# MGI-tech-bioinformatics/SuperPlus

Hardware: AMD Instinct MI355X
Metric: k-mers/s (DF createDict stage: trim + canonical k-mer count + solid filter + spectrum + adjacency) (higher is better)
Workload: dtype u64

## Files before the change

superplus_amd/csrc/dfk.hip:

```cpp
#include "../../include/dfk.h"
#include "dfk_kernels.h"

#include <algorithm>
#include <chrono>
#include <cstdarg>
#include <cstdio>
#include <cstdlib>
#include <cstring>
#include <atomic>
#include <fcntl.h>
#include <functional>
#include <new>
#include <string>
#include <sys/mman.h>
#include <sys/stat.h>
#include <unistd.h>
#include <condition_variable>
#include <memory>
#include <mutex>
#include <thread>
#include <vector>

using namespace dfk;

// ... 279 lines not shown
    DevBuf ctr; int rc = c->alloc(ctr, 32, "trim counters"); if (rc) return rc;
    HIP_TRY(hipMemsetAsync(ctr.p, 0, 32, c->stream));
    rc = c->alloc(c->good_len, sizeof(uint32_t) * in.n_reads, "goodLens", true); if (rc) return rc;
    if (in.n_reads) {
        unsigned grid = (unsigned)std::min<uint64_t>((in.n_reads + 255) / 256, 8192);
        hipLaunchKernelGGL(HIP_KERNEL_NAME(k_trim<K>), dim3(grid), dim3(256), 0, c->stream,
                           in.pq, in.pq_off, in.pq_bytes, in.base_off, in.packed_bytes, in.read_len, in.n_reads, c->cfg.min_qual, (uint32_t*)c->good_len.p,
                           (unsigned long long*)ctr.p, (unsigned int*)((char*)ctr.p + 8),
                           (unsigned long long*)((char*)ctr.p + 16));
        HIP_TRY(hipGetLastError());
    }
    uint64_t h[3] = {0, 0, 0};
    HIP_TRY(hipMemcpyAsync(h, ctr.p, 24, hipMemcpyDeviceToHost, c->stream));
    HIP_TRY(hipStreamSynchronize(c->stream));
    c->release(ctr);
    if ((uint32_t)h[1]) return fail(DFK_E_INPUT, "malformed input: an offset table is not monotone or runs past its array, a PQVec stream is broken, or its length differs from read_len");
    if (h[2] == 0) return fail(DFK_E_NOGOOD, "Looks like your input data have almost no good bases.");
    *n_inst = h[0];
    return 0;
}

int device_scan(dfk_ctx* c, const uint64_t* in, uint64_t* out, uint64_t n)
{
    constexpr uint64_t PER = (uint64_t)SCAN_THREADS * SCAN_ITEMS;
    if (n == 0) return 0;
    const uint64_t nblk = (n + PER - 1) / PER;
    if (nblk == 1) {
        hipLaunchKernelGGL(k_scan_blocks, dim3(1), dim3(SCAN_THREADS), 0, c->stream, in, out, n, (uint64_t*)nullptr);
        HIP_TRY(hipGetLastError());
        return 0;
    }
    DevBuf sums; int rc = c->alloc(sums, nblk * 8, "scan block sums"); if (rc) return rc;
    hipLaunchKernelGGL(k_scan_blocks, dim3((unsigned)nblk), dim3(SCAN_THREADS), 0, c->stream, in, out, n, (uint64_t*)sums.p);
    HIP_TRY(hipGetLastError());
    rc = device_scan(c, (const uint64_t*)sums.p, (uint64_t*)sums.p, nblk); if (rc) return rc;
    hipLaunchKernelGGL(k_scan_add, dim3((unsigned)nblk), dim3(SCAN_THREADS), 0, c->stream, out, n, (const uint64_t*)sums.p);
    HIP_TRY(hipGetLastError());
    HIP_TRY(hipStreamSynchronize(c->stream));
    c->release(sums);
    return 0;
}

struct BucketTable {
    uint32_t log2_nb = 0;
    DevBuf acc;
    DevBuf summ;
    DevBuf classes;
    DevBuf ovf_list; uint64_t n_ovf = 0;
    DevBuf class_hist;
    std::vector<uint64_t> h_class;
    uint64_t n_records = 0, n_inst = 0;
};
struct Partition {
    DevBuf records, base, ipre, items;
    uint64_t n_records = 0, n_inst = 0, n_items = 0;
    uint64_t nb = 0;
};

template <int K>
PartParams part_params(const dfk_ctx* c, uint32_t log2_nb, uint32_t log2_world, int64_t read_id0, uint32_t sub_lo, uint32_t sub_n)
{
    const uint32_t M = c->cfg.minimizer_len;
    return PartParams{M, (uint32_t)K - M + 1, log2_nb, log2_world, read_id0, sub_lo, sub_n,
                      sweep_class_mask(sub_lo, sub_n, log2_nb - log2_world)};
}

int table_totals(dfk_ctx* c, const DevBuf& acc, uint64_t nb, uint64_t* n_records, uint64_t* n_inst)
{
    DevBuf tot; int rc = c->alloc(tot, 16, "bucket totals"); if (rc) return rc;
    HIP_TRY(hipMemsetAsync(tot.p, 0, 16, c->stream));
    hipLaunchKernelGGL(k_sum_acc, dim3(1024), dim3(256), 0, c->stream, (const unsigned long long*)acc.p, nb, (unsigned long long*)tot.p);
    HIP_TRY(hipGetLastError());
    uint64_t h[2];
    HIP_TRY(hipMemcpyAsync(h, tot.p, 16, hipMemcpyDeviceToHost, c->stream));
    HIP_TRY(hipStreamSynchronize(c->stream));
    c->release(tot);
    *n_records = h[0]; *n_inst = h[1];
    return 0;
}

struct ScanJob {
    PartParams pp; uint64_t nb = 0, n_bins = 0, ovf_cap = 0; bool by_class = false, ranged = false;
    DevBuf ovf_tmp, d_n;
    std::vector<std::pair<hipEvent_t, hipEvent_t>> ev;
    ~ScanJob() { for (auto& e : ev) { (void)hipEventDestroy(e.first); (void)hipEventDestroy(e.second); } }
};

template <int K> bool scan_takes_ranges(const dfk_ctx* c) { return c->cfg.minimizer_len == 16; }

template <int K>
int scan_begin(dfk_ctx* c, const Inputs& in, uint32_t log2_world, int64_t read_id0, BucketTable* T, bool by_class, ScanJob* J)
{
    J->pp = part_params<K>(c, T->log2_nb, log2_world, read_id0, 0, 1u << (T->log2_nb - log2_world));
    J->nb = 1ull << T->log2_nb; J->by_class = by_class;
    int rc = 0;
    J->n_bins = 2ull * (PART_CLASSES << log2_world);
    if (by_class) { rc = c->alloc(T->class_hist, J->n_bins * 8, "class counters", true); if (rc) return rc; HIP_TRY(hipMemsetAsync(T->class_hist.p, 0, J->n_bins * 8, c->stream)); }
    else { rc = c->alloc(T->acc, J->nb * 8, "bucket counters", true); if (rc) return rc; }
    rc = c->alloc(T->summ, std::max<uint64_t>(1, in.n_reads) * 16, "run summaries", true); if (rc) return rc;
    rc = c->alloc(T->classes, std::max<uint64_t>(1, in.n_reads) * 4, "read bucket classes", true); if (rc) return rc;
    if (!by_class) HIP_TRY(hipMemsetAsync(T->acc.p, 0, J->nb * 8, c->stream));
    J->ovf_cap = in.n_reads / 16 + 1024;
    rc = c->alloc(J->ovf_tmp, J->ovf_cap * 4, "overflow read list (scratch)"); if (rc) return rc;
    rc = c->alloc(J->d_n, 16, "overflow read count"); if (rc) return rc;
    HIP_TRY(hipMemsetAsync(J->d_n.p, 0, 16, c->stream));
    return 0;
}

template <int K>
int scan_range(dfk_ctx* c, const Inputs& in, BucketTable* T, ScanJob* J, uint64_t r0, uint64_t r1)
{
    if (r1 <= r0) return 0;
    const PartParams& pp = J->pp;
    const bool by_class = J->by_class;
    unsigned grid = (unsigned)((r1 - r0 + PART_THREADS - 1) / PART_THREADS);
    static const unsigned scan_blocks = getenv("DFK_SCAN_BLOCKS") ? (unsigned)atoi(getenv("DFK_SCAN_BLOCKS")) : 0;
    if (by_class) grid = std::min<unsigned>(grid, (scan_blocks ? scan_blocks : 128u) * (unsigned)c->prop.multiProcessorCount);
    else if (scan_blocks) grid = std::min<unsigned>(grid, scan_blocks * (unsigned)c->prop.multiProcessorCount);
    const size_t lds_a = (sizeof(uint32_t) + 1) * pp.W * PART_THREADS + sizeof(uint32_t) * PART_RING * PART_THREADS + (by_class ? J->n_bins * 4 : 0);
    hipEvent_t e0, e1;
    HIP_TRY(hipEventCreate(&e0)); HIP_TRY(hipEventCreate(&e1));
    J->ev.emplace_back(e0, e1);
    HIP_TRY(hipEventRecord(e0, c->stream));
    if (scan_takes_ranges<K>(c)) {
        const size_t lds_r = sizeof(uint32_t) * (PART_RING + SUMMARY_RUNS) * PART_THREADS + (by_class ? J->n_bins * 4 : 0);
        hipLaunchKernelGGL(HIP_KERNEL_NAME(k_scan_count<K, 16>), dim3(grid), dim3(PART_THREADS), lds_r, c->stream,
                           in.packed, in.packed_bytes, in.base_off, (const uint32_t*)c->good_len.p, r0, r1, pp,
                           (unsigned long long*)T->acc.p, (unsigned long long*)T->class_hist.p, (unsigned long long*)J->d_n.p, J->ovf_cap,
                           (uint32_t*)J->ovf_tmp.p, (uint4*)T->summ.p, (uint32_t*)T->classes.p);
    } else {
        if (r0 != 0 || r1 != in.n_reads) return fail(DFK_E_STATE, "the general scan takes every read at once");
        hipLaunchKernelGGL(HIP_KERNEL_NAME(k_partition<K, false>), dim3(grid), dim3(PART_THREADS), lds_a, c->stream,
                           in.packed, in.packed_bytes, in.base_off, (const uint32_t*)c->good_len.p, in.bc,
                           (int64_t)c->cfg.ign_bc_below, in.n_reads, pp, (unsigned long long*)T->acc.p, (unsigned long long*)T->class_hist.p,
                           (unsigned long long*)J->d_n.p, J->ovf_cap, (uint4*)J->ovf_tmp.p, (uint4*)T->summ.p,
                           (const uint32_t*)nullptr, (uint64_t)0, (const uint64_t*)nullptr, (uint32_t*)T->classes.p);
    }
    HIP_TRY(hipGetLastError());
    HIP_TRY(hipEventRecord(e1, c->stream));
    return 0;
}

template <int K>
int scan_end(dfk_ctx* c, const Inputs& in, uint64_t n_inst, BucketTable* T, ScanJob* J)
{
    int rc = 0;
    T->n_ovf = 0;
    if (in.n_reads) {
        HIP_TRY(hipMemcpyAsync(&T->n_ovf, J->d_n.p, 8, hipMemcpyDeviceToHost, c->stream));
        HIP_TRY(hipStreamSynchronize(c->stream));
        if (T->n_ovf > J->ovf_cap) {
            c->release(J->ovf_tmp);
            rc = c->alloc(J->ovf_tmp, in.n_reads * 4, "overflow read list (scratch)"); if (rc) return rc;
            HIP_TRY(hipMemsetAsync(J->d_n.p, 0, 16, c->stream));
            hipLaunchKernelGGL(k_select_overflow, dim3((unsigned)std::min<uint64_t>((in.n_reads + 255) / 256, 8192)), dim3(256), 0, c->stream,
                               (const uint4*)T->summ.p, in.n_reads, (uint32_t*)J->ovf_tmp.p, (unsigned long long*)J->d_n.p);
            HIP_TRY(hipGetLastError());
            HIP_TRY(hipMemcpyAsync(&T->n_ovf, J->d_n.p, 8, hipMemcpyDeviceToHost, c->stream));
            HIP_TRY(hipStreamSynchronize(c->stream));
        }
        if (T->n_ovf) {
            rc = c->alloc(T->ovf_list, T->n_ovf * 4, "overflow read list", true); if (rc) return rc;
            HIP_TRY(hipMemcpyAsync(T->ovf_list.p, J->ovf_tmp.p, T->n_ovf * 4, hipMemcpyDeviceToDevice, c->stream));
            HIP_TRY(hipStreamSynchronize(c->stream));
        }
    }
    c->release(J->ovf_tmp); c->release(J->d_n);
    HIP_TRY(hipStreamSynchronize(c->stream));
    float ms = 0;
    for (auto& e : J->ev) { float m = 0; if (hipEventElapsedTime(&m, e.first, e.second) == hipSuccess) ms += m; }
    c->st.ms_part_count = ms; c->st.reserved[6] = J->ev.size();
    TRACE("%llu of %llu reads have more than %d runs", (unsigned long long)T->n_ovf, (unsigned long long)in.n_reads, SUMMARY_RUNS);
    if (J->by_class) {
        T->h_class.assign(J->n_bins, 0);
        HIP_TRY(hipMemcpyAsync(T->h_class.data(), T->class_hist.p, J->n_bins * 8, hipMemcpyDeviceToHost, c->stream));
        HIP_TRY(hipStreamSynchronize(c->stream));
        T->n_records = T->n_inst = 0;
        for (uint64_t i = 0; i < J->n_bins / 2; ++i) { T->n_records += T->h_class[i]; T->n_inst += T->h_class[J->n_bins / 2 + i]; }
    } else { rc = table_totals(c, T->acc, J->nb, &T->n_records, &T->n_inst); if (rc) return rc; }
    TRACE("partition count pass done (%llu buckets, %llu records%s)", (unsigned long long)J->nb, (unsigned long long)T->n_records, J->ev.size() > 1 ? ", in ranges under the upload" : "");
    if (T->n_inst != n_inst)
        return fail(DFK_E_HIP, "partition count pass saw %llu instances, trim saw %llu%s",
                    (unsigned long long)T->n_inst, (unsigned long long)n_inst,
                    (n_inst - T->n_inst) % (1ull << 32) == 0 ? " (a fine bucket with 2^32 or more instances: its counter keeps 32 bits)" : "");
    c->st.n_records = T->n_records; c->st.n_buckets = J->nb;
    return 0;
}

template <int K>
int partition_count(dfk_ctx* c, const Inputs& in, uint64_t n_inst, uint32_t log2_world, int64_t read_id0, BucketTable* T, bool by_class = false)
{
    ScanJob J;
    int rc = scan_begin<K>(c, in, log2_world, read_id0, T, by_class, &J); if (rc) return rc;
    rc = scan_range<K>(c, in, T, &J, 0, in.n_reads); if (rc) return rc;
    return scan_end<K>(c, in, n_inst, T, &J);
}

int pass_tables(dfk_ctx* c, const DevBuf& acc, uint32_t log2_sub, uint32_t world, uint32_t sub_lo, uint32_t sub_n, uint64_t budget, Partition* P)
{
    P->nb = (uint64_t)world * sub_n;
    const uint64_t nb = P->nb;
    DevBuf rec, inst, flags, idx;
    int rc = c->alloc(rec, (nb + 1) * 8, "bucket record counts"); if (rc) return rc;
    rc = c->alloc(inst, (nb + 1) * 8, "bucket instance counts"); if (rc) return rc;
    rc = c->alloc(P->base, (nb + 1) * 8, "bucket bases"); if (rc) return rc;
    rc = c->alloc(P->ipre, (nb + 1) * 8, "bucket instance prefix"); if (rc) return rc;
    const unsigned g1 = (unsigned)((nb + 1 + 255) / 256);
    hipLaunchKernelGGL(k_slice, dim3(g1), dim3(256), 0, c->stream, (const unsigned long long*)acc.p, log2_sub, sub_lo, sub_n, nb,
                       (uint64_t*)rec.p, (uint64_t*)inst.p);
    HIP_TRY(hipGetLastError());
    rc = device_scan(c, (const uint64_t*)rec.p, (uint64_t*)P->base.p, nb + 1); if (rc) return rc;
    rc = device_scan(c, (const uint64_t*)inst.p, (uint64_t*)P->ipre.p, nb + 1); if (rc) return rc;
    rc = c->alloc(flags, (nb + 1) * 8, "item flags"); if (rc) return rc;
    rc = c->alloc(idx, (nb + 1) * 8, "item index"); if (rc) return rc;
    hipLaunchKernelGGL(k_item_flags, dim3(g1), dim3(256), 0, c->stream, (const uint64_t*)P->ipre.p, nb, budget, (uint64_t*)flags.p);
    HIP_TRY(hipGetLastError());
    rc = device_scan(c, (const uint64_t*)flags.p, (uint64_t*)idx.p, nb + 1); if (rc) return rc;
    uint64_t tot[3];
    HIP_TRY(hipMemcpyAsync(&tot[0], (const uint64_t*)P->base.p + nb, 8, hipMemcpyDeviceToHost, c->stream));
    HIP_TRY(hipMemcpyAsync(&tot[1], (const uint64_t*)P->ipre.p + nb, 8, hipMemcpyDeviceToHost, c->stream));
    HIP_TRY(hipMemcpyAsync(&tot[2], (const uint64_t*)idx.p + nb, 8, hipMemcpyDeviceToHost, c->stream));
    HIP_TRY(hipStreamSynchronize(c->stream));
    P->n_records = tot[0]; P->n_inst = tot[1]; P->n_items = tot[2];
    rc = c->alloc(P->items, std::max<uint64_t>(1, P->n_items) * sizeof(ItemRange), "work items"); if (rc) return rc;
    hipLaunchKernelGGL(k_item_pairs, dim3((unsigned)((nb + 255) / 256)), dim3(256), 0, c->stream, (const uint64_t*)flags.p,
                       (const uint64_t*)idx.p, nb, (ItemRange*)P->items.p);
    HIP_TRY(hipGetLastError());
    HIP_TRY(hipStreamSynchronize(c->stream));
    c->release(rec); c->release(inst); c->release(flags); c->release(idx);
    return 0;
// ... 1641 lines not shown
```

superplus_amd/csrc/dfk_kernels.h:

```cpp
#pragma once
#include <type_traits>
#include "dfk_device.h"

namespace dfk {

template <int K>
__global__ void __launch_bounds__(256)
k_trim(const uint8_t* __restrict__ pq, const uint64_t* __restrict__ pq_off, uint64_t pq_nbytes,
       const uint64_t* __restrict__ base_off, uint64_t packed_bytes, const uint32_t* __restrict__ read_len,
       uint64_t n_reads, uint32_t min_qual, uint32_t* __restrict__ good_len,
       unsigned long long* __restrict__ n_inst, unsigned int* __restrict__ bad,
       unsigned long long* __restrict__ sum_good)
{
    unsigned long long mine = 0, good = 0;
    bool any_bad = false;
    for (uint64_t r = (uint64_t)blockIdx.x * blockDim.x + threadIdx.x; r < n_reads; r += (uint64_t)gridDim.x * blockDim.x) {
        uint32_t gl = 0;
        uint64_t p = pq_off[r], end = pq_off[r + 1];
        uint32_t idx = 0, run = 0;
        const uint64_t b0 = base_off[r], b1 = base_off[r + 1];
        bool ok = p <= end && end <= pq_nbytes && b0 <= b1 && b1 <= packed_bytes && b1 - b0 >= ((uint64_t)read_len[r] + 3) / 4;
        if (!ok) end = p;
        while (p < end) {
            uint32_t nQs = pq[p];
// ... 259 lines not shown
        }
        arr[bi * PART_THREADS + tid] = h;
        if (++bi == W) {
            uint32_t run = h, ri = W - 1;
            if (!WRITE) sidx[(W - 1) * PART_THREADS + tid] = (uint8_t)(W - 1);
            for (int i0 = (int)W - 2; i0 >= 0; i0 -= 8) {
                uint32_t v[8];
#pragma unroll
                for (int k = 0; k < 8; ++k) v[k] = i0 - k >= 0 ? arr[(i0 - k) * PART_THREADS + tid] : 0u;
#pragma unroll
                for (int k = 0; k < 8; ++k) {
                    const int i = i0 - k;
                    if (i >= 0) {
                        const bool lt = v[k] < run;
                        run = lt ? v[k] : run;
                        arr[i * PART_THREADS + tid] = run;
                        if (!WRITE) { ri = lt ? (uint32_t)i : ri; sidx[i * PART_THREADS + tid] = (uint8_t)ri; }
                    }
                }
            }
            bi = 0;
        }
        if (bi + 1 < W) sfx_next = arr[(bi + 1) * PART_THREADS + tid];
    }
    close_run();
    if (!WRITE) {
        const uint64_t lo = sum_lo | (qn <= (uint32_t)SUMMARY_RUNS ? qn : SUMMARY_OVERFLOW), hi = sum_hi;
        summaries[r] = uint4{(uint32_t)lo, (uint32_t)(lo >> 32), (uint32_t)hi, (uint32_t)(hi >> 32)};
        if (read_classes) read_classes[r] = cmask;
        if (qn > (uint32_t)SUMMARY_RUNS && bucket_cur) {
            const unsigned long long at = atomicAdd(bucket_cur, 1ull);
            if (at < n_out) reinterpret_cast<uint32_t*>(records)[at] = (uint32_t)r;
        }
    }
    if (WRITE) {
        for (uint32_t e = 0; e < qn; ++e) {
            uint32_t a = queue[(2 * e) * PART_THREADS + tid], b = queue[(2 * e + 1) * PART_THREADS + tid];
            const uint64_t dst = place(b);
            if (dst != ~0ull) emit_record<K>(words, n_words, bit0, a & 0xFFFFu, a >> 16, b, gl, tag, dst, records);
        }
    }
}

template <int K, bool WRITE>
__global__ void __launch_bounds__(PART_THREADS)
k_partition(const uint8_t* __restrict__ packed, uint64_t packed_bytes, const uint64_t* __restrict__ base_off,
            const uint32_t* __restrict__ good_len, const int32_t* __restrict__ bc, int64_t ign_bc_below,
            uint64_t n_reads, PartParams pp,
            unsigned long long* __restrict__ bucket_acc,
            unsigned long long* __restrict__ class_hist,
            unsigned long long* __restrict__ bucket_cur,
            uint64_t n_out,
            uint4* __restrict__ records,
            uint4* __restrict__ summaries,
            const uint32_t* __restrict__ read_list,
            uint64_t n_list,
            const uint64_t* __restrict__ slice_base,
            uint32_t* __restrict__ read_classes)
{
    extern __shared__ uint32_t smem[];
    uint32_t* lh = nullptr;
    const uint32_t n_bins = 2u * (PART_CLASSES << pp.log2_world);
    if (!WRITE && class_hist) {
        lh = reinterpret_cast<uint32_t*>(reinterpret_cast<uint8_t*>(smem) + 5 * pp.W * PART_THREADS + 4 * PART_RING * PART_THREADS);
        for (uint32_t i = threadIdx.x; i < n_bins; i += PART_THREADS) lh[i] = 0;
        __syncthreads();
    }
    const uint64_t n_work = (WRITE && read_list) ? n_list : n_reads;
    for (uint64_t r0 = (uint64_t)blockIdx.x * PART_THREADS; r0 < n_work; r0 += (uint64_t)gridDim.x * PART_THREADS)
        partition_read<K, WRITE>(r0 + threadIdx.x, smem, lh, packed, packed_bytes, base_off, good_len, bc, ign_bc_below, n_reads, pp,
                                 bucket_acc, bucket_cur, n_out, records, summaries, read_list, n_list, slice_base, read_classes);
    if (lh) {
        __syncthreads();
        for (uint32_t i = threadIdx.x; i < n_bins; i += PART_THREADS) if (lh[i]) atomicAdd(&class_hist[i], (unsigned long long)lh[i]);
    }
}

template <int I, int N, class F>
__device__ __forceinline__ void static_for(F&& f)
{
    if constexpr (I < N) { f(std::integral_constant<int, I>{}); static_for<I + 1, N>(f); }
}

template <int K, int M>
__global__ void __launch_bounds__(PART_THREADS)
k_scan_count(const uint8_t* __restrict__ packed, uint64_t packed_bytes, const uint64_t* __restrict__ base_off,
             const uint32_t* __restrict__ good_len, uint64_t r_first, uint64_t n_reads , PartParams pp,
             unsigned long long* __restrict__ bucket_acc, unsigned long long* __restrict__ class_hist,
             unsigned long long* __restrict__ ovf_count, uint64_t ovf_cap, uint32_t* __restrict__ ovf_list,
             uint4* __restrict__ summaries, uint32_t* __restrict__ read_classes)
{
    constexpr int W = K - M + 1;
    constexpr uint32_t mmask = M == 16 ? 0xFFFFFFFFu : ((1u << (2 * M)) - 1u);
    constexpr uint32_t rsh = 2 * (M - 1);
    constexpr int RUNS = SUMMARY_RUNS;
    extern __shared__ uint32_t smem[];
    uint32_t* ring = smem;
    uint32_t* runb = smem + PART_RING * PART_THREADS;
    uint32_t* lh = nullptr;
    const uint32_t n_bins = 2u * (PART_CLASSES << pp.log2_world);
    if (class_hist) {
        lh = runb + RUNS * PART_THREADS;
        for (uint32_t i = threadIdx.x; i < n_bins; i += PART_THREADS) lh[i] = 0;
        __syncthreads();
    }
    const int tid = threadIdx.x;
    const uint32_t* words = reinterpret_cast<const uint32_t*>(packed);
    const uint64_t n_words = (packed_bytes + 3) >> 2;
    const uint32_t log2_local = pp.log2_nb - pp.log2_world;
    for (uint64_t r0 = r_first + (uint64_t)blockIdx.x * PART_THREADS; r0 < n_reads; r0 += (uint64_t)gridDim.x * PART_THREADS) {
        const uint64_t r = r0 + tid;
        const uint32_t gl = r < n_reads ? good_len[r] : 0;
        const bool live = gl >= (uint32_t)K + 1;
        uint32_t qn = 0, cmask = 0;
        uint64_t sum_lo = 0, sum_hi = 0;
        if (live) {
            const uint64_t bit0 = base_off[r] * 8;
            uint64_t wi = bit0 >> 5, filled_to = wi;
            auto fill = [&]() {
                uint32_t w[PART_RING];
#pragma unroll
                for (int k = 0; k < PART_RING; ++k) w[k] = filled_to + k < n_words ? words[filled_to + k] : 0u;
#pragma unroll
                for (int k = 0; k < PART_RING; ++k) ring[((filled_to + k) & (PART_RING - 1)) * PART_THREADS + tid] = w[k];
                filled_to += PART_RING;
            };
            fill();
            uint32_t wbits = ring[(wi & (PART_RING - 1)) * PART_THREADS + tid], wpos = (uint32_t)bit0 & 31u;
            auto next_base = [&]() -> uint32_t {
                const uint32_t b = (wbits >> wpos) & 3u;
                wpos += 2;
                if (wpos == 32) { wpos = 0; ++wi; if (wi == filled_to) fill(); wbits = ring[(wi & (PART_RING - 1)) * PART_THREADS + tid]; }
                return b;
            };
            uint32_t f = 0, rc = 0;
            for (int j = 0; j < M - 1; ++j) { const uint32_t b = next_base(); f = ((f << 2) | b) & mmask; rc = (rc >> 2) | ((3u - b) << rsh); }
            const uint32_t n_mmers = gl - M + 1;
            uint32_t arr[W], sidxw[(W + 3) / 4];
            auto sidx_get = [&](int i) -> uint32_t { return (sidxw[i >> 2] >> (8 * (i & 3))) & 255u; };
            auto sidx_set = [&](int i, uint32_t v) { const uint32_t sh = 8u * (uint32_t)(i & 3); sidxw[i >> 2] = (sidxw[i >> 2] & ~(255u << sh)) | (v << sh); };
#pragma unroll
            for (int i = 0; i < (W + 3) / 4; ++i) sidxw[i] = 0;
            uint32_t P = 0, Pi = 0;
            uint32_t cur_b = 0, cur_nk = 0, cur_rel = 0;
            auto close_run = [&]() {
                if (qn < (uint32_t)RUNS) {
                    runb[qn * PART_THREADS + tid] = cur_b;
                    const uint64_t fld = cur_nk | (cur_rel << 6);
                    const uint32_t b = 8u + 12u * qn;
                    if (b < 64u) { sum_lo |= fld << b; if (b > 52u) sum_hi |= fld >> (64u - b); } else sum_hi |= fld << (b - 64u);
                } else {
                    if (lh) { const uint32_t bin = class_bin(cur_b, pp); atomicAdd(&lh[bin], 1u); atomicAdd(&lh[(PART_CLASSES << pp.log2_world) + bin], cur_nk); }
                    else atomicAdd(&bucket_acc[cur_b], (1ull << 32) | cur_nk);
                    cmask |= 1u << sweep_class_of(cur_b & ((1u << log2_local) - 1u), log2_local);
                }
                ++qn;
            };
            for (uint32_t t0 = 0; t0 < n_mmers; t0 += W) {
                static_for<0, W>([&](auto bi_c) {
                    constexpr int bi = decltype(bi_c)::value;
                    if (t0 + (uint32_t)bi < n_mmers) {
                        const uint32_t b = next_base();
                        f = ((f << 2) | b) & mmask;
                        rc = (rc >> 2) | ((3u - b) << rsh);
                        const uint32_t h = mmer_hash(f < rc ? f : rc);
                        const bool newmin = bi == 0 || h < P;
                        P = newmin ? h : P;
                        Pi = newmin ? (uint32_t)bi : Pi;
                        const bool first = t0 == 0;
                        if (!first || bi == W - 1) {
                            uint32_t mv = P;
                            bool older = false;
                            if constexpr (bi != W - 1) { older = arr[bi + 1] < mv; mv = older ? arr[bi + 1] : mv; }
                            const uint32_t bucket = bucket_of(mv, pp);
                            const bool open = first || bucket != cur_b || cur_nk == (uint32_t)KTraits<K>::NK_MAX;
                            if (open) {
                                if (!first) close_run();
                                cur_b = bucket; cur_nk = 1;
                                cur_rel = (bi != W - 1 && older) ? sidx_get(bi + 1 < W ? bi + 1 : 0) - (uint32_t)bi - 1u : (uint32_t)(W - 1 - bi) + Pi;
                            } else ++cur_nk;
                        }
                        arr[bi] = h;
                        if (bi == W - 1) {
                            uint32_t run = h, ri = W - 1;
                            sidx_set(W - 1, W - 1);
                            static_for<0, W - 1>([&](auto j_c) {
                                constexpr int i = W - 2 - decltype(j_c)::value;
                                const bool lt = arr[i] < run; run = lt ? arr[i] : run; arr[i] = run; ri = lt ? (uint32_t)i : ri; sidx_set(i, ri);
                            });
                        }
                    }
                });
            }
            close_run();
        }
        const uint32_t mine = min(qn, (uint32_t)RUNS);
        for (uint32_t i = 0; __ballot(i < mine) != 0ull; ++i) {
            if (i < mine) {
                const uint32_t cb = runb[i * PART_THREADS + tid];
                const uint32_t bfld = 8u + 12u * i;
                const uint32_t nk = (uint32_t)(bfld + 12 <= 64 ? sum_lo >> bfld : bfld >= 64 ? sum_hi >> (bfld - 64) : (sum_lo >> bfld) | (sum_hi << (64 - bfld))) & 63u;
                if (lh) { const uint32_t bin = class_bin(cb, pp); atomicAdd(&lh[bin], 1u); atomicAdd(&lh[(PART_CLASSES << pp.log2_world) + bin], nk); }
                else atomicAdd(&bucket_acc[cb], (1ull << 32) | nk);
                cmask |= 1u << sweep_class_of(cb & ((1u << log2_local) - 1u), log2_local);
            }
        }
        if (r < n_reads) {
            const uint64_t lo = sum_lo | (qn <= (uint32_t)SUMMARY_RUNS ? qn : SUMMARY_OVERFLOW);
            summaries[r] = uint4{(uint32_t)lo, (uint32_t)(lo >> 32), (uint32_t)sum_hi, (uint32_t)(sum_hi >> 32)};
            if (read_classes) read_classes[r] = cmask;
        }
        if (qn > (uint32_t)SUMMARY_RUNS) {
            const unsigned long long at = atomicAdd(ovf_count, 1ull);
            if (at < ovf_cap) ovf_list[at] = (uint32_t)r;
        }
    }
    if (lh) {
        __syncthreads();
        for (uint32_t i = threadIdx.x; i < n_bins; i += PART_THREADS) if (lh[i]) atomicAdd(&class_hist[i], (unsigned long long)lh[i]);
    }
}

constexpr int SLICE_READS = 16;
template <int K, bool EMIT, typename F>
__device__ __forceinline__ void for_each_run_in_pass(uint64_t r, const uint8_t* __restrict__ packed, uint64_t packed_bytes,
                                                     const uint64_t* __restrict__ base_off, const PartParams& pp,
                                                     const uint4* __restrict__ summaries, F&& f)
{
    const uint4 sm = summaries[r];
    const uint32_t n = sm.x & 15u;
    if (n == 0 || n == SUMMARY_OVERFLOW) return;
    const uint32_t* words = reinterpret_cast<const uint32_t*>(packed);
    const uint64_t n_words = (packed_bytes + 3) >> 2;
    const uint64_t bit0 = base_off[r] * 8;
    const uint32_t M = pp.M;
    const uint32_t mmask = M == 16 ? 0xFFFFFFFFu : ((1u << (2 * M)) - 1u);
    const uint64_t lo = (uint64_t)sm.x | ((uint64_t)sm.y << 32), hi = (uint64_t)sm.z | ((uint64_t)sm.w << 32);
    uint32_t s0 = 0;
#pragma unroll
    for (int i = 0; i < SUMMARY_RUNS; ++i) {
        if ((uint32_t)i < n) {
            constexpr int B0 = 8;
            const int b = B0 + 12 * i;
            const uint32_t fld = (uint32_t)(b + 12 <= 64 ? lo >> b : b >= 64 ? hi >> (b - 64) : (lo >> b) | (hi << (64 - b))) & 0xFFFu;
            const uint32_t nk = fld & 63u, rel = fld >> 6;
            const uint64_t bo = bit0 + 2ull * (s0 + rel);
            const uint64_t wi = bo >> 5;
            const uint32_t w0 = words[wi], w1 = wi + 1 < n_words ? words[wi + 1] : 0u;
            const uint32_t x = alignbit(w1, w0, (uint32_t)bo & 31u) & mmask;
            uint32_t y = __brev(x);
            y = ((y >> 1) & 0x55555555u) | ((y & 0x55555555u) << 1);
            const uint32_t fw = y >> (32 - 2 * M), rcv = ~x & mmask;
            const uint32_t bucket = bucket_of(mmer_hash(fw < rcv ? fw : rcv), pp);
            const uint32_t lb = pass_local(bucket, pp);
            if (lb != 0xFFFFFFFFu) f(s0, nk, lb, bucket >> (pp.log2_nb - pp.log2_world), bit0, (uint32_t)i + 1 == n);
            s0 += nk;
        }
    }
}

template <int K>
__global__ void __launch_bounds__(256)
k_scatter_slices(const uint8_t* __restrict__ packed, uint64_t packed_bytes, const uint64_t* __restrict__ base_off,
                 const uint32_t* __restrict__ good_len, const int32_t* __restrict__ bc, int64_t ign_bc_below,
                 uint64_t n_reads, PartParams pp, const uint4* __restrict__ summaries, const uint32_t* __restrict__ read_classes,
                 const uint64_t* __restrict__ slice_base,
                 unsigned long long* __restrict__ slice_fill,
                 uint4* __restrict__ records)
{
    __shared__ uint32_t cnt[256];
    __shared__ unsigned long long at[256];
    __shared__ uint16_t list[256 * SLICE_READS];
    __shared__ uint32_t n_list;
    const uint32_t world = 1u << pp.log2_world;
    const int lane = threadIdx.x & 63;
    const uint64_t r_block = (uint64_t)blockIdx.x * 256 * SLICE_READS;
    if (threadIdx.x < world) cnt[threadIdx.x] = 0;
    if (threadIdx.x == 0) n_list = 0;
    __syncthreads();
#pragma unroll
    for (int j = 0; j < SLICE_READS; ++j) {
        const uint32_t rel = 256u * j + threadIdx.x;
        const uint64_t r = r_block + rel;
        const bool hit = r < n_reads && (!read_classes || (read_classes[r] & pp.class_mask) != 0u);
        const unsigned long long mk = __ballot(hit);
        uint32_t w = 0;
        if (lane == 0 && mk) w = atomicAdd(&n_list, (uint32_t)__popcll(mk));
        w = __builtin_amdgcn_readfirstlane(w);
        if (hit) list[w + __popcll(mk & ((1ull << lane) - 1ull))] = (uint16_t)rel;
    }
    __syncthreads();
    const uint32_t n = n_list;
    for (uint32_t i = threadIdx.x; i < n; i += 256)
        for_each_run_in_pass<K, false>(r_block + list[i], packed, packed_bytes, base_off, pp, summaries,
                                       [&](uint32_t, uint32_t, uint32_t, uint32_t owner, uint64_t, bool) { atomicAdd(&cnt[owner], 1u); });
    __syncthreads();
    if (threadIdx.x < world) {
        const uint32_t m = cnt[threadIdx.x];
        at[threadIdx.x] = slice_base[threadIdx.x] + (m ? atomicAdd(&slice_fill[threadIdx.x], (unsigned long long)m) : 0ull);
        cnt[threadIdx.x] = 0;
    }
    __syncthreads();
    const uint32_t* words = reinterpret_cast<const uint32_t*>(packed);
// ... 1542 lines not shown
```

Baseline: 58.49 billion.

## Stage scan run keys by class and count via LDS sub-slice histograms

Instead of issuing a global 64-bit atomic per run into the bucket counter table, the ranged scan kernel stages run keys in LDS and flushes them into per-class global key arrays. A pipeline of follow-up kernels (sub-slice histogram, prefix scan, partition, per-sub-slice LDS count) then accumulates the bucket counters with shared-memory atomics and a single plain add per bucket. The aim is to remove scattered global atomic traffic over a large table. In exchange it adds multi-GB scratch buffers, extra block-wide synchronisation in the scan kernel, and several extra passes over the keys. It is only enabled when the estimated runs per read is at least 3.5.

```diff
diff --git a/superplus_amd/csrc/dfk.hip b/superplus_amd/csrc/dfk.hip
--- a/superplus_amd/csrc/dfk.hip
+++ b/superplus_amd/csrc/dfk.hip
@@ -385,6 +385,9 @@
 struct ScanJob {
     PartParams pp; uint64_t nb = 0, n_bins = 0, ovf_cap = 0; bool by_class = false, ranged = false;
     DevBuf ovf_tmp, d_n;
+    bool keyed = false; uint32_t n_cls = 0, n_sub = 0, sb = 0; uint64_t piece_reads = 0;
+    ScanKeys sk{};
+    DevBuf keys, keys2, fill, sub;
     std::vector<std::pair<hipEvent_t, hipEvent_t>> ev;
     ~ScanJob() { for (auto& e : ev) { (void)hipEventDestroy(e.first); (void)hipEventDestroy(e.second); } }
 };
@@ -407,6 +410,62 @@
     rc = c->alloc(J->ovf_tmp, J->ovf_cap * 4, "overflow read list (scratch)"); if (rc) return rc;
     rc = c->alloc(J->d_n, 16, "overflow read count"); if (rc) return rc;
     HIP_TRY(hipMemsetAsync(J->d_n.p, 0, 16, c->stream));
+    const double runs = in.n_reads ? 1.0 + 2.0 * std::max(0.0, 4.0 * (double)in.packed_bytes / (double)in.n_reads - K + 1) / (J->pp.W + 1) : 0.0;
+    J->keyed = !by_class && scan_takes_ranges<K>(c) && in.n_reads && (runs >= 3.5 || getenv("DFK_SCAN_KEY_PIECE"));
+    if (J->keyed) {
+        const uint32_t lb = T->log2_nb, cb = std::min<uint32_t>(6, lb);
+        J->sk.ib = lb - cb; J->n_cls = 1u << cb;
+        J->sb = std::min(KEY_SUB_BITS, J->sk.ib); J->n_sub = 1u << (J->sk.ib - J->sb);
+        const double per_read = 1.25 * runs;
+        constexpr uint64_t KEY_SCRATCH_MAX = 16ull << 30;
+        const uint64_t want = 8ull * (uint64_t)(per_read * (double)in.n_reads) + 8ull * J->n_cls;
+        const uint64_t room = std::min<uint64_t>(std::min(want, KEY_SCRATCH_MAX), c->largest_allocatable() / 3);
+        J->sk.cap = std::max<uint64_t>(1024, room / 8 / J->n_cls);
+        J->piece_reads = std::max<uint64_t>(PART_THREADS, (uint64_t)((double)(J->sk.cap * J->n_cls) / per_read));
+        if (const char* e = getenv("DFK_SCAN_KEY_PIECE")) J->piece_reads = std::max<uint64_t>(1, std::min<uint64_t>(J->piece_reads, strtoull(e, nullptr, 10)));
+        const uint64_t n_subs = (uint64_t)J->n_cls * J->n_sub;
+        rc = c->alloc(J->keys, J->sk.cap * J->n_cls * 4, "run keys (scratch)"); if (rc) return rc;
+        rc = c->alloc(J->keys2, J->sk.cap * J->n_cls * 4, "run keys by sub-slice (scratch)"); if (rc) return rc;
+        rc = c->alloc(J->fill, J->n_cls * 8, "run key slice fills (scratch)"); if (rc) return rc;
+        rc = c->alloc(J->sub, (3 * n_subs + 1) * 8, "run key sub-slices (scratch)"); if (rc) return rc;
+        J->sk.keys = (uint32_t*)J->keys.p; J->sk.fill = (unsigned long long*)J->fill.p;
+        TRACE("run keys: %u classes of %llu keys, %u sub-slices each, pieces of %llu reads", J->n_cls, (unsigned long long)J->sk.cap,
+              J->n_sub, (unsigned long long)J->piece_reads);
+    }
+    return 0;
+}
+
+template <int K>
+int scan_keys_piece(dfk_ctx* c, const Inputs& in, BucketTable* T, ScanJob* J, uint64_t r0, uint64_t r1)
+{
+    static const unsigned scan_blocks = getenv("DFK_SCAN_BLOCKS") ? (unsigned)atoi(getenv("DFK_SCAN_BLOCKS")) : 0;
+    const unsigned cus = (unsigned)c->prop.multiProcessorCount;
+    const unsigned grid = (unsigned)std::min<uint64_t>((r1 - r0 + PART_THREADS - 1) / PART_THREADS, (uint64_t)(scan_blocks ? scan_blocks : 128u) * cus);
+    const uint64_t n_subs = (uint64_t)J->n_cls * J->n_sub;
+    auto* cnt = (unsigned long long*)J->sub.p;
+    auto* off = cnt + n_subs;
+    auto* cur = off + n_subs + 1;
+    HIP_TRY(hipMemsetAsync(J->fill.p, 0, J->n_cls * 8, c->stream));
+    HIP_TRY(hipMemsetAsync(cnt, 0, n_subs * 8, c->stream));
+    const size_t lds = sizeof(uint32_t) * (PART_RING + SUMMARY_RUNS) * PART_THREADS + SCAN_STAGE_LDS;
+    hipLaunchKernelGGL(HIP_KERNEL_NAME(k_scan_count<K, 16, true>), dim3(grid), dim3(PART_THREADS), lds, c->stream,
+                       in.packed, in.packed_bytes, in.base_off, (const uint32_t*)c->good_len.p, r0, r1, J->pp,
+                       (unsigned long long*)T->acc.p, (unsigned long long*)nullptr, (unsigned long long*)J->d_n.p, J->ovf_cap,
+                       (uint32_t*)J->ovf_tmp.p, (uint4*)T->summ.p, (uint32_t*)T->classes.p, J->sk);
+    HIP_TRY(hipGetLastError());
+    const dim3 per_class(std::max(1u, 16u * cus / J->n_cls), J->n_cls);
+    const uint32_t sh = 6 + J->sb;
+    hipLaunchKernelGGL(k_keys_subcount, per_class, dim3(256), J->n_sub * 4, c->stream,
+                       (const uint32_t*)J->keys.p, (const unsigned long long*)J->fill.p, J->sk.cap, sh, J->n_sub, cnt);
+    HIP_TRY(hipGetLastError());
+    hipLaunchKernelGGL(k_keys_offsets, dim3(1), dim3(1024), 0, c->stream, (const unsigned long long*)cnt, (uint32_t)n_subs, off, cur);
+    HIP_TRY(hipGetLastError());
+    hipLaunchKernelGGL(k_keys_partition, per_class, dim3(256), J->n_sub * 12, c->stream,
+                       (const uint32_t*)J->keys.p, (const unsigned long long*)J->fill.p, J->sk.cap, sh, J->n_sub, cur, (uint32_t*)J->keys2.p);
+    HIP_TRY(hipGetLastError());
+    hipLaunchKernelGGL(k_keys_count, dim3((unsigned)n_subs), dim3(1024), 0, c->stream,
+                       (const uint32_t*)J->keys2.p, (const unsigned long long*)off, J->sb, (unsigned long long*)T->acc.p);
+    HIP_TRY(hipGetLastError());
     return 0;
 }
 
@@ -425,12 +484,16 @@
     HIP_TRY(hipEventCreate(&e0)); HIP_TRY(hipEventCreate(&e1));
     J->ev.emplace_back(e0, e1);
     HIP_TRY(hipEventRecord(e0, c->stream));
-    if (scan_takes_ranges<K>(c)) {
+    if (J->keyed) {
+        for (uint64_t p0 = r0; p0 < r1; p0 += J->piece_reads) {
+            int rc = scan_keys_piece<K>(c, in, T, J, p0, std::min(r1, p0 + J->piece_reads)); if (rc) return rc;
+        }
+    } else if (scan_takes_ranges<K>(c)) {
         const size_t lds_r = sizeof(uint32_t) * (PART_RING + SUMMARY_RUNS) * PART_THREADS + (by_class ? J->n_bins * 4 : 0);
-        hipLaunchKernelGGL(HIP_KERNEL_NAME(k_scan_count<K, 16>), dim3(grid), dim3(PART_THREADS), lds_r, c->stream,
+        hipLaunchKernelGGL(HIP_KERNEL_NAME(k_scan_count<K, 16, false>), dim3(grid), dim3(PART_THREADS), lds_r, c->stream,
                            in.packed, in.packed_bytes, in.base_off, (const uint32_t*)c->good_len.p, r0, r1, pp,
                            (unsigned long long*)T->acc.p, (unsigned long long*)T->class_hist.p, (unsigned long long*)J->d_n.p, J->ovf_cap,
-                           (uint32_t*)J->ovf_tmp.p, (uint4*)T->summ.p, (uint32_t*)T->classes.p);
+                           (uint32_t*)J->ovf_tmp.p, (uint4*)T->summ.p, (uint32_t*)T->classes.p, ScanKeys{});
     } else {
         if (r0 != 0 || r1 != in.n_reads) return fail(DFK_E_STATE, "the general scan takes every read at once");
         hipLaunchKernelGGL(HIP_KERNEL_NAME(k_partition<K, false>), dim3(grid), dim3(PART_THREADS), lds_a, c->stream,
@@ -449,6 +512,7 @@
 {
     int rc = 0;
     T->n_ovf = 0;
+    c->release(J->keys); c->release(J->keys2); c->release(J->fill); c->release(J->sub);
     if (in.n_reads) {
         HIP_TRY(hipMemcpyAsync(&T->n_ovf, J->d_n.p, 8, hipMemcpyDeviceToHost, c->stream));
         HIP_TRY(hipStreamSynchronize(c->stream));
diff --git a/superplus_amd/csrc/dfk_kernels.h b/superplus_amd/csrc/dfk_kernels.h
--- a/superplus_amd/csrc/dfk_kernels.h
+++ b/superplus_amd/csrc/dfk_kernels.h
@@ -365,18 +365,29 @@
     if constexpr (I < N) { f(std::integral_constant<int, I>{}); static_for<I + 1, N>(f); }
 }
 
-template <int K, int M>
+struct ScanKeys {
+    uint32_t* keys;
+    unsigned long long* fill;
+    uint64_t cap;
+    uint32_t ib;
+};
+constexpr int SCAN_STAGE = 1792;
+constexpr uint32_t KEY_SUB_BITS = 14;
+constexpr uint32_t KEY_TILE = 16384;
+
+template <int K, int M, bool KEYS>
 __global__ void __launch_bounds__(PART_THREADS)
 k_scan_count(const uint8_t* __restrict__ packed, uint64_t packed_bytes, const uint64_t* __restrict__ base_off,
              const uint32_t* __restrict__ good_len, uint64_t r_first, uint64_t n_reads , PartParams pp,
              unsigned long long* __restrict__ bucket_acc, unsigned long long* __restrict__ class_hist,
              unsigned long long* __restrict__ ovf_count, uint64_t ovf_cap, uint32_t* __restrict__ ovf_list,
-             uint4* __restrict__ summaries, uint32_t* __restrict__ read_classes)
+             uint4* __restrict__ summaries, uint32_t* __restrict__ read_classes, ScanKeys sk)
 {
     constexpr int W = K - M + 1;
     constexpr uint32_t mmask = M == 16 ? 0xFFFFFFFFu : ((1u << (2 * M)) - 1u);
     constexpr uint32_t rsh = 2 * (M - 1);
     constexpr int RUNS = SUMMARY_RUNS;
+    static_assert(KTraits<K>::NK_MAX < 64, "nk takes the key's six low bits");
     extern __shared__ uint32_t smem[];
     uint32_t* ring = smem;
     uint32_t* runb = smem + PART_RING * PART_THREADS;
@@ -388,6 +399,32 @@
         __syncthreads();
     }
     const int tid = threadIdx.x;
+    uint32_t* st_key = runb + RUNS * PART_THREADS;
+    unsigned long long* st_base = reinterpret_cast<unsigned long long*>(st_key + SCAN_STAGE);
+    uint32_t* st_h = reinterpret_cast<uint32_t*>(st_base + PART_CLASSES);
+    uint32_t* st_n = st_h + PART_CLASSES;
+    uint8_t* st_cls = reinterpret_cast<uint8_t*>(st_n + 1);
+    const uint32_t n_cls = 1u << (pp.log2_nb - sk.ib);
+    if constexpr (KEYS) {
+        if (tid < PART_CLASSES) st_h[tid] = 0;
+        if (tid == 0) *st_n = 0;
+        __syncthreads();
+    }
+    auto flush = [&]() {
+        const uint32_t n = *st_n;
+        if (tid < (int)n_cls) { const uint32_t h = st_h[tid]; if (h) st_base[tid] = atomicAdd(&sk.fill[tid], (unsigned long long)h); st_h[tid] = 0; }
+        __syncthreads();
+        for (uint32_t j = tid; j < n; j += PART_THREADS) {
+            const uint32_t key = st_key[j], cls = st_cls[j];
+            const unsigned long long at = st_base[cls] + atomicAdd(&st_h[cls], 1u);
+            if (at < sk.cap) sk.keys[cls * sk.cap + at] = key;
+            else atomicAdd(&bucket_acc[(cls << sk.ib) | (key >> 6)], (1ull << 32) | (key & 63u));
+        }
+        __syncthreads();
+        if (tid < (int)n_cls) st_h[tid] = 0;
+        if (tid == 0) *st_n = 0;
+        __syncthreads();
+    };
     const uint32_t* words = reinterpret_cast<const uint32_t*>(packed);
     const uint64_t n_words = (packed_bytes + 3) >> 2;
     const uint32_t log2_local = pp.log2_nb - pp.log2_world;
@@ -478,14 +515,36 @@
             close_run();
         }
         const uint32_t mine = min(qn, (uint32_t)RUNS);
-        for (uint32_t i = 0; __ballot(i < mine) != 0ull; ++i) {
-            if (i < mine) {
-                const uint32_t cb = runb[i * PART_THREADS + tid];
+        for (uint32_t i = 0; KEYS ? __syncthreads_or(i < mine) != 0 : __ballot(i < mine) != 0ull; ++i) {
+            const bool has = i < mine;
+            uint32_t cb = 0, nk = 0;
+            if (has) {
+                cb = runb[i * PART_THREADS + tid];
                 const uint32_t bfld = 8u + 12u * i;
-                const uint32_t nk = (uint32_t)(bfld + 12 <= 64 ? sum_lo >> bfld : bfld >= 64 ? sum_hi >> (bfld - 64) : (sum_lo >> bfld) | (sum_hi << (64 - bfld))) & 63u;
-                if (lh) { const uint32_t bin = class_bin(cb, pp); atomicAdd(&lh[bin], 1u); atomicAdd(&lh[(PART_CLASSES << pp.log2_world) + bin], nk); }
-                else atomicAdd(&bucket_acc[cb], (1ull << 32) | nk);
+                nk = (uint32_t)(bfld + 12 <= 64 ? sum_lo >> bfld : bfld >= 64 ? sum_hi >> (bfld - 64) : (sum_lo >> bfld) | (sum_hi << (64 - bfld))) & 63u;
+                if constexpr (!KEYS) {
+                    if (lh) { const uint32_t bin = class_bin(cb, pp); atomicAdd(&lh[bin], 1u); atomicAdd(&lh[(PART_CLASSES << pp.log2_world) + bin], nk); }
+                    else atomicAdd(&bucket_acc[cb], (1ull << 32) | nk);
+                }
                 cmask |= 1u << sweep_class_of(cb & ((1u << log2_local) - 1u), log2_local);
+            }
+            if constexpr (KEYS) {
+                const uint64_t m = __ballot(has);
+                if (m) {
+                    const uint32_t rk = __builtin_amdgcn_mbcnt_hi((uint32_t)(m >> 32), __builtin_amdgcn_mbcnt_lo((uint32_t)m, 0u));
+                    const int lead = __ffsll((unsigned long long)m) - 1;
+                    uint32_t at = 0;
+                    if (has && rk == 0) at = atomicAdd(st_n, (uint32_t)__popcll(m));
+                    at = __shfl(at, lead) + rk;
+                    if (has) {
+                        const uint32_t cls = cb >> sk.ib;
+                        st_key[at] = ((cb & ((1u << sk.ib) - 1u)) << 6) | nk;
+                        st_cls[at] = (uint8_t)cls;
+                        atomicAdd(&st_h[cls], 1u);
+                    }
+                }
+                __syncthreads();
+                if (*st_n > (uint32_t)(SCAN_STAGE - PART_THREADS)) flush();
             }
         }
         if (r < n_reads) {
@@ -498,10 +557,92 @@
             if (at < ovf_cap) ovf_list[at] = (uint32_t)r;
         }
     }
+    if constexpr (KEYS) { __syncthreads(); if (*st_n) flush(); }
     if (lh) {
         __syncthreads();
         for (uint32_t i = threadIdx.x; i < n_bins; i += PART_THREADS) if (lh[i]) atomicAdd(&class_hist[i], (unsigned long long)lh[i]);
     }
+}
+constexpr size_t SCAN_STAGE_LDS = (sizeof(uint32_t) + 1) * SCAN_STAGE + (sizeof(unsigned long long) + sizeof(uint32_t)) * PART_CLASSES + sizeof(uint32_t);
+
+__global__ void __launch_bounds__(256)
+k_keys_subcount(const uint32_t* __restrict__ keys, const unsigned long long* __restrict__ fill, uint64_t cap, uint32_t sh ,
+                uint32_t n_sub, unsigned long long* __restrict__ sub_cnt)
+{
+    extern __shared__ uint32_t lh[];
+    const uint32_t c = blockIdx.y;
+    for (uint32_t i = threadIdx.x; i < n_sub; i += blockDim.x) lh[i] = 0;
+    __syncthreads();
+    const uint64_t n = min((uint64_t)fill[c], cap);
+    const uint32_t* k = keys + c * cap;
+    for (uint64_t i = (uint64_t)blockIdx.x * blockDim.x + threadIdx.x; i < n; i += (uint64_t)gridDim.x * blockDim.x) atomicAdd(&lh[k[i] >> sh], 1u);
+    __syncthreads();
+    for (uint32_t i = threadIdx.x; i < n_sub; i += blockDim.x) if (lh[i]) atomicAdd(&sub_cnt[(uint64_t)c * n_sub + i], (unsigned long long)lh[i]);
+}
+
+__global__ void __launch_bounds__(1024)
+k_keys_offsets(const unsigned long long* __restrict__ cnt, uint32_t n, unsigned long long* __restrict__ off, unsigned long long* __restrict__ cur)
+{
+    __shared__ unsigned long long part[1024];
+    const uint32_t tid = threadIdx.x, per = (n + 1023) / 1024;
+    const uint32_t lo = min(n, tid * per), hi = min(n, lo + per);
+    unsigned long long s = 0;
+    for (uint32_t i = lo; i < hi; ++i) s += cnt[i];
+    part[tid] = s;
+    __syncthreads();
+    for (uint32_t d = 1; d < 1024; d <<= 1) {
+        const unsigned long long v = tid >= d ? part[tid - d] : 0ull;
+        __syncthreads();
+        part[tid] += v;
+        __syncthreads();
+    }
+    unsigned long long run = part[tid] - s;
+    for (uint32_t i = lo; i < hi; ++i) { off[i] = run; cur[i] = run; run += cnt[i]; }
+    if (tid == 1023) off[n] = part[1023];
+}
+
+__global__ void __launch_bounds__(256)
+k_keys_partition(const uint32_t* __restrict__ keys, const unsigned long long* __restrict__ fill, uint64_t cap, uint32_t sh,
+                 uint32_t n_sub, unsigned long long* __restrict__ cur, uint32_t* __restrict__ out)
+{
+    extern __shared__ unsigned long long lds64[];
+    unsigned long long* base = lds64;
+    uint32_t* lh = reinterpret_cast<uint32_t*>(lds64 + n_sub);
+    const uint32_t c = blockIdx.y;
+    const uint64_t n = min((uint64_t)fill[c], cap);
+    const uint32_t* k = keys + c * cap;
+    unsigned long long* cc = cur + (uint64_t)c * n_sub;
+    for (uint64_t t0 = (uint64_t)blockIdx.x * KEY_TILE; t0 < n; t0 += (uint64_t)gridDim.x * KEY_TILE) {
+        const uint64_t t1 = min(n, t0 + KEY_TILE);
+        for (uint32_t i = threadIdx.x; i < n_sub; i += blockDim.x) lh[i] = 0;
+        __syncthreads();
+        for (uint64_t i = t0 + threadIdx.x; i < t1; i += blockDim.x) atomicAdd(&lh[k[i] >> sh], 1u);
+        __syncthreads();
+        for (uint32_t i = threadIdx.x; i < n_sub; i += blockDim.x) { if (lh[i]) base[i] = atomicAdd(&cc[i], (unsigned long long)lh[i]); lh[i] = 0; }
+        __syncthreads();
+        for (uint64_t i = t0 + threadIdx.x; i < t1; i += blockDim.x) {
+            const uint32_t key = k[i], s = key >> sh;
+            out[base[s] + atomicAdd(&lh[s], 1u)] = key;
+        }
+        __syncthreads();
+    }
+}
+
+__global__ void __launch_bounds__(1024)
+k_keys_count(const uint32_t* __restrict__ part, const unsigned long long* __restrict__ off, uint32_t sb, unsigned long long* __restrict__ bucket_acc)
+{
+    __shared__ unsigned long long t[1u << KEY_SUB_BITS];
+    const uint32_t s = blockIdx.x, nt = 1u << sb, m = nt - 1u;
+    for (uint32_t i = threadIdx.x; i < nt; i += blockDim.x) t[i] = 0;
+    __syncthreads();
+    const uint64_t a = off[s], b = off[s + 1];
+    for (uint64_t i = a + threadIdx.x; i < b; i += blockDim.x) {
+        const uint32_t key = part[i];
+        atomicAdd(&t[(key >> 6) & m], (1ull << 32) | (key & 63u));
+    }
+    __syncthreads();
+    unsigned long long* dst = bucket_acc + ((uint64_t)s << sb);
+    for (uint32_t i = threadIdx.x; i < nt; i += blockDim.x) if (t[i]) dst[i] += t[i];
 }
 
 constexpr int SLICE_READS = 16;
```

Measured after the change: 59.94 billion, median of 6. 1.02x the previous value.
